# ctu-mrs/space_filling_forest_star

Hardware: AMD Instinct MI355X
Metric: accepted node expansions/sec + collision checks/sec, dense_3D 6-DoF (higher is better)
Workload: dtype f64

## Files before the change

space_filling_forest_star_amd/csrc/forest_dev.cpp:

```cpp
#include <algorithm>
#include <chrono>
#include <cmath>
#include <cstdio>
#include <cstdlib>
#include <cstring>
#include <thread>
#include <vector>

#include "engine.h"
#include "sff_geom.h"

namespace sff {

#define HIPCHK(x) hip_check((x), #x)
using Clock = std::chrono::steady_clock;
static double ms_since(Clock::time_point t0) { return std::chrono::duration<double, std::milli>(Clock::now() - t0).count(); }

static uint64_t next_pow2(uint64_t v) {
  uint64_t p = 1;
  while (p < v) p <<= 1;
  return p;
}

bool Forest::device_eligible() const {
// ... 1573 lines not shown
        if (g[24]) fprintf(stderr, "[sffgpu k_star_tail, sections of a sample's pass (STAR_PASS_TRACE build)] us: first loads %.1f views %.1f evaluate %.1f (of it requests %.1f) "
                           "loops %.1f writes %.1f\n", g[24] / ps / 100.0, g[25] / ps / 100.0, (g[26] + g[27]) / ps / 100.0, g[27] / ps / 100.0, g[28] / ps / 100.0, g[29] / ps / 100.0);
      }
    }
    const double r = (double)std::max<unsigned long long>(1ULL, k.prof[6]);
    if (d.kc_trace.p) {
      const size_t nw = (size_t)cfg.wave / 64 + 2;
      std::vector<unsigned long long> tr(nw * 8);
      HIPCHK(hipMemcpy(tr.data(), d.kc_trace.p, nw * 64, hipMemcpyDeviceToHost));
      unsigned long long t0 = ~0ULL;
      size_t used = 0;
      for (size_t w = 0; w < nw; ++w) if (tr[8 * w]) { t0 = std::min(t0, tr[8 * w]); used = w + 1; }
      static const char* names[8] = {"start", "walk done", "count published", "stamps posted", "lower counts in (ids)", "lower stamps in", "lower owned counts in", "end"};
      for (int k = 0; k < 8 && used; ++k) {
        std::vector<double> v;
        for (size_t w = 0; w < used; ++w) if (tr[8 * w + k]) v.push_back((double)(tr[8 * w + k] - t0) / 100.0);
        if (v.empty()) continue;
        std::vector<double> sv = v;
        std::sort(sv.begin(), sv.end());
        fprintf(stderr, "[sffgpu k_commit trace, %zu workgroups] %-24s us after the first start: min %.1f median %.1f max %.1f | first wg %.1f last wg %.1f\n",
                used, names[k], sv.front(), sv[sv.size() / 2], sv.back(), v.front(), v.back());
      }
    }
    fprintf(stderr, "[sffgpu k_commit us/commit, last workgroup] walks + waits for earlier samples %.1f (%.2f polls, max %llu) "
            "lower workgroups' counts %.1f borders %.1f control block %.1f | dependent/round %.0f\n", k.prof[0] / r / 100.0, k.prof[5] / r,
            (unsigned long long)k.prof[7], k.prof[1] / r / 100.0, k.prof[2] / r / 100.0, k.prof[3] / r / 100.0,
            (double)k.n_unsettled / r);
#ifdef SFFK_CI_TRACE
    {
      std::vector<unsigned long long> tr(4096 * 8);
      sffk::debug_ci_trace(tr.data());
      unsigned long long t0 = ~0ULL, tend = 0;
      for (int w = 0; w < 4096; ++w) if (tr[8 * w]) { t0 = std::min(t0, tr[8 * w]); tend = std::max(tend, tr[8 * w + 7]); }
      struct It { double start, broad, end; int nc, smp, items, wave; double entry, pre; };
      std::vector<It> its;
      int waves = 0, n_pose_items = 0;
      double pose_us = 0, pose_max = 0;
      for (int w = 0; w < 4096; ++w) {
        if (!tr[8 * w]) continue;
        ++waves;
        { const unsigned long long pp = tr[8 * w + 6] >> 8; n_pose_items += (int)(pp & 0xff); pose_us += (double)(pp >> 8) / 100.0; if ((pp & 0xff) && (double)(pp >> 8) / 100.0 > pose_max) pose_max = (double)(pp >> 8) / 100.0; tr[8 * w + 6] &= 0xff; }
        if (!tr[8 * w + 6]) continue;
        its.push_back({(tr[8 * w + 1] - t0) / 100.0, tr[8 * w + 2] >= tr[8 * w + 1] ? (tr[8 * w + 2] - t0) / 100.0 : -1.0, (tr[8 * w + 3] - t0) / 100.0,
                       (int)tr[8 * w + 4], (int)(tr[8 * w + 5] & 0xff), (int)tr[8 * w + 6], w, (tr[8 * w] - t0) / 100.0, ((tr[8 * w + 5] >> 8) - t0) / 100.0});
      }
      std::sort(its.begin(), its.end(), [](const It& a, const It& b) { return a.end > b.end; });
      fprintf(stderr, "[sffgpu k_collide_items trace] %d waves, %zu with items, kernel %.1f us (first start -> last end)\n", waves, its.size(), (tend - t0) / 100.0);
      for (size_t k = 0; k < its.size() && k < 12; ++k)
        fprintf(stderr, "  wave %4d: entry %.1f preamble done %.1f | items %d | first item: start %.1f broad done %.1f end %.1f us | candidates %d masked samples %d\n",
                its[k].wave, its[k].entry, its[k].pre, its[k].items, its[k].start, its[k].broad, its[k].end, its[k].nc, its[k].smp);
      {
        std::vector<double> e, p, st, en;
        for (const It& i : its) { e.push_back(i.entry); p.push_back(i.pre); st.push_back(i.start); en.push_back(i.end); }
        auto q = [](std::vector<double> v, double f) { std::sort(v.begin(), v.end()); return v.empty() ? 0.0 : v[(size_t)(f * (v.size() - 1))]; };
        fprintf(stderr, "  entry min/med/max %.1f %.1f %.1f | preamble done %.1f %.1f %.1f | first item start %.1f %.1f %.1f | end %.1f %.1f %.1f\n",
                q(e, 0), q(e, .5), q(e, 1), q(p, 0), q(p, .5), q(p, 1), q(st, 0), q(st, .5), q(st, 1), q(en, 0), q(en, .5), q(en, 1));
      }
      double sum_b = 0, sum_n = 0; int nb = 0;
      for (const It& i : its) if (i.broad >= 0) { sum_b += i.broad - i.start; sum_n += i.end - i.broad; ++nb; }
      if (nb) fprintf(stderr, "  first items with a broad phase: %d, avg broad %.1f us, avg after-broad %.1f us\n", nb, sum_b / nb, sum_n / nb);
      fprintf(stderr, "  pose items: %d, avg %.1f us, longest per wave %.1f us\n", n_pose_items, n_pose_items ? pose_us / n_pose_items : 0.0, pose_max);
    }
#endif
#ifdef SFFK_DEBUG_COUNTERS
    unsigned long long g[16];
    sffk::debug_counters(g);
    const double items = (double)std::max<unsigned long long>(1ULL, g[1]);
    fprintf(stderr, "[sffgpu exact kernel, per masked chunk] chunks %llu (with work %llu, with candidates %llu) flushes %.2f "
            "candidates %.1f | us: setup %.2f hierarchy %.2f narrow %.2f | per wave total %.1f us over %llu waves\n",
            g[0], g[1], g[2], g[3] / items, g[7] / items, g[4] / items / 100.0, g[5] / items / 100.0, g[6] / items / 100.0,
            (double)g[8] / (double)std::max<unsigned long long>(1ULL, g[9]) / 100.0, g[9]);
    fprintf(stderr, "[sffgpu exact kernel, narrow phase per chunk with candidates] us: staging %.2f culls %.2f exact steps %.2f (the rest: pair formation) | "
            "touching (sample, candidate) pairs %.2f\n", g[10] / 100.0 / (double)std::max<unsigned long long>(1ULL, g[2]),
            g[11] / 100.0 / (double)std::max<unsigned long long>(1ULL, g[2]), g[13] / 100.0 / (double)std::max<unsigned long long>(1ULL, g[2]),
            (double)g[14] / (double)std::max<unsigned long long>(1ULL, g[2]));
    unsigned long long q[16];
    sffk::debug_counters_query(q);
    const double qw = (double)std::max<unsigned long long>(1ULL, q[0]);
    fprintf(stderr, "[sffgpu query kernel, per sampled wave] us: grid scan %.2f classify %.2f cull %.2f (flushes %.2f) | live %.2f "
            "pairs/live %.1f survivors/live %.2f\n", q[1] / qw / 100.0, q[2] / qw / 100.0, q[3] / qw / 100.0, q[4] / qw / 100.0,
            q[7] / qw, (double)q[5] / (double)std::max<unsigned long long>(1ULL, q[7]),
            (double)q[6] / (double)std::max<unsigned long long>(1ULL, q[7]));
    fprintf(stderr, "[sffgpu block query kernel] us per sampled workgroup: samples %.2f | cells+lists %.2f | 2nd list %.2f | exact %.2f | classify %.2f | cull %.2f | flush %.2f\n",
            q[1] / qw / 100.0, q[2] / qw / 100.0, q[3] / qw / 100.0, q[4] / qw / 100.0, q[5] / qw / 100.0, q[6] / qw / 100.0, q[7] / qw / 100.0);
    fprintf(stderr, "[sffgpu block query kernel] shader clock over the sampled workgroups' lifetimes: %.0f MHz (lifetime %.2f us)\n",
            100.0 * (double)q[10] / (double)std::max<unsigned long long>(1ULL, q[11]), q[11] / qw / 100.0);
#endif
  }
}

}
```

space_filling_forest_star_amd/csrc/kernels.hip:

```cpp
#include <hip/hip_runtime.h>
#include <stdint.h>
#include <stdlib.h>
#include <string.h>
#include "kernels.h"
#include <algorithm>
#include "sff_geom.h"
#include "kernels_dev.h"
#include "star_pass_dev.h"
#include "prio_heap_dev.h"

namespace sffk {

using namespace sffg;


__global__ __launch_bounds__(256) void k_sample_steer(SampleLaunch P) {
  const int i = blockIdx.x * blockDim.x + threadIdx.x;
  sample_steer_one(i, P);
}

__device__ __forceinline__ float wrapf(float d) {
  const float PI_F = 3.14159274f;
  if (d < -PI_F) return d + 2.0f * PI_F;
  if (d >= PI_F) return d - 2.0f * PI_F;
// ... 1374 lines not shown
  xform(R, p, rob.center, c);
}

#ifndef SEG_WAVES
#define SEG_WAVES 4
#endif
#ifndef SHARE_WORK
#define SHARE_WORK 192
#endif
#ifndef SHARE_POSE_MIN
#define SHARE_POSE_MIN 8
#endif
#define SHARE_IDLE (1 << 30)
__device__ __forceinline__ int share_block(int nc) { return nc >= 64 ? 4 : (nc >= 24 ? 2 : 1); }
struct ShareSlot {
  unsigned long long sk;
  int nc, done_k, minhit, seg, chunk, kind;
  unsigned long long mask;
  double a[6], b[6], R[9];
};
struct ShareArea {
  ShareSlot slot[SEG_WAVES];
  int done_waves;
};
__device__ __forceinline__ unsigned long long lds_load64(const unsigned long long* p) {
  return __hip_atomic_load(p, __ATOMIC_RELAXED, __HIP_MEMORY_SCOPE_WORKGROUP);
}
__device__ __forceinline__ int lds_load32(const int* p) { return __hip_atomic_load(p, __ATOMIC_RELAXED, __HIP_MEMORY_SCOPE_WORKGROUP); }
__device__ void share_init(ShareArea& sh) {
  if (threadIdx.x < SEG_WAVES) { sh.slot[threadIdx.x].sk = (unsigned long long)SHARE_IDLE; sh.slot[threadIdx.x].nc = 0; }
  if (threadIdx.x == 0) sh.done_waves = 0;
}

__device__ bool pose_block(const EnvView& env, const RobotView& rob, const double* rtri, double* stage, const int32_t* cand,
                           int k0, int kc, const double* p, const double* R, const double* c, double rr, int lane) {
  bool hit = false;
  stage_candidates(env, cand, k0, kc, lane, stage);
  for (int r0 = 0; r0 < rob.n_tri && !hit; r0 += 64) {
    const int r = r0 + lane;
    double Q[9];
    const bool have = r < rob.n_tri;
    if (have)
      for (int v = 0; v < 3; ++v) xform(R, p, rtri + 9 * r + 3 * v, Q + 3 * v);
    bool lane_hit = false;
    for (int k = 0; k < kc; ++k) {
      const double* sb = stage + k * STAGE_TRI;
      if (plane_clear(sb + 6, c, rr)) continue;
      if (have && !lane_hit) {
        if (tri_box_overlap(sb, sb + 3, Q)) lane_hit = sat17(sb + 11, Q);
      }
    }
    hit = __any(lane_hit);
  }
  __builtin_amdgcn_wave_barrier();
  return hit;
}

__device__ bool pose_exact(const EnvView& env, const RobotView& rob, const double* rtri, int32_t* stack, int32_t* cand,
                           double* stage, const double* p, const double* R, const double* c, int lane, ShareArea* share = nullptr) {
  double qlo[3], qhi[3];
  double rr = rob.radius * (1 + 1e-9) + 1e-9 * (fabs(c[0]) + fabs(c[1]) + fabs(c[2]) + 1);
  for (int k = 0; k < 3; ++k) { qlo[k] = c[k] - rr; qhi[k] = c[k] + rr; }

  WaveStack st{stack, 0, stack + STACK_CAP};
  bool overflow;
  int nc = collect_candidates(env, qlo, qhi, lane, st, cand, CAND_CAP, &overflow);
  bool hit = false;
  if (overflow) {
    for (int r0 = 0; r0 < rob.n_tri && !hit; r0 += 64) {
      const int r = r0 + lane;
      double Q[9];
      const bool have = r < rob.n_tri;
      if (have)
        for (int v = 0; v < 3; ++v) xform(R, p, rtri + 9 * r + 3 * v, Q + 3 * v);
      bool lane_hit = false;
      for (int t = 0; t < env.n_tri; ++t) {
        if (have && !lane_hit) {
          const double* b = env.tri_box + 6 * (size_t)t;
          if (tri_box_overlap(b, b + 3, Q)) lane_hit = sat17(env.tri + 9 * (size_t)t, Q);
        }
      }
      hit = __any(lane_hit);
    }
  } else {
    const bool shared = share && nc >= SHARE_POSE_MIN;
    ShareSlot* const hs = shared ? &share->slot[threadIdx.x >> 6] : nullptr;
    unsigned seq = 0;
    if (shared && lane == 0) {
      seq = (unsigned)(hs->sk >> 32) + 1u;
      hs->nc = nc; hs->done_k = 0; hs->minhit = 0x7fffffff; hs->kind = 1;
      for (int k = 0; k < 6; ++k) hs->a[k] = p[k];
      for (int k = 0; k < 3; ++k) hs->b[k] = c[k];
      for (int k = 0; k < 9; ++k) hs->R[k] = R[k];
      __threadfence_block();
      __hip_atomic_store(&hs->sk, (unsigned long long)seq << 32, __ATOMIC_RELAXED, __HIP_MEMORY_SCOPE_WORKGROUP);
    }
    const int blk = shared ? share_block(nc) : STAGE_N;
    for (int knext = 0; !hit; knext += STAGE_N) {
      int k0 = knext;
      if (shared) {
        int seen = 0x7fffffff;
        if (lane == 0) {
          k0 = (int)(unsigned)(atomicAdd(&hs->sk, (unsigned long long)blk) & 0xffffffffULL);
          seen = lds_load32(&hs->minhit);
        }
        k0 = __builtin_amdgcn_readfirstlane(k0);
        seen = __builtin_amdgcn_readfirstlane(seen);
        if (k0 >= nc) break;
        const int kc = nc - k0 < blk ? nc - k0 : blk;
        const bool h = seen == 0 ? true : pose_block(env, rob, rtri, stage, cand, k0, kc, p, R, c, rr, lane);
        if (lane == 0) {
          if (h) atomicMin(&hs->minhit, 0);
          atomicAdd(&hs->done_k, kc);
        }
        continue;
      }
      if (k0 >= nc) break;
      const int kc = nc - k0 < blk ? nc - k0 : blk;
      hit = pose_block(env, rob, rtri, stage, cand, k0, kc, p, R, c, rr, lane);
    }
    if (shared) {
      int out = 0;
      if (lane == 0) {
        while (lds_load32(&hs->done_k) < nc) __builtin_amdgcn_s_sleep(2);
        out = lds_load32(&hs->minhit);
        __hip_atomic_store(&hs->sk, ((unsigned long long)seq << 32) | (unsigned long long)SHARE_IDLE, __ATOMIC_RELAXED, __HIP_MEMORY_SCOPE_WORKGROUP);
      }
      hit = __builtin_amdgcn_readfirstlane(out) == 0;
    }
  }
  return hit;
}

__global__ __launch_bounds__(64 * POSE_WAVES) void k_collide_poses(EnvView env, RobotView rob,
                                                                   const double* __restrict__ pos6, int n,
                                                                   const int32_t* __restrict__ live_flags,
                                                                   uint8_t* __restrict__ hit_out, int explicit_rt) {
  extern __shared__ double lds_d[];
  double* rtri = lds_d;
  const int wave = threadIdx.x >> 6, lane = threadIdx.x & 63;
  double* stage = rtri + (size_t)rob.n_tri * 9 + (size_t)wave * STAGE_DOUBLES;
  int32_t* ibase = reinterpret_cast<int32_t*>(rtri + (size_t)rob.n_tri * 9 + (size_t)POSE_WAVES * STAGE_DOUBLES);
  int32_t* stack = ibase + wave * (STACK_CAP + TG_HASH);
  int32_t* cand = ibase + POSE_WAVES * (STACK_CAP + TG_HASH) + wave * CAND_CAP;
  const int pose = blockIdx.x * POSE_WAVES + wave;
  bool need = false;
  double p[6], R[9], c[3] = {0, 0, 0};
  if (pose < n) {
    const bool run = !live_flags || (live_flags[pose] & 3) == 1;
    if (run && env.n_tri != 0) {
      if (explicit_rt) {
        const double* rt = pos6 + 12 * (size_t)pose;
        for (int k = 0; k < 9; ++k) R[k] = rt[k];
        for (int k = 0; k < 3; ++k) { p[k] = rt[9 + k]; p[3 + k] = 0; }
        need = !surely_clear(env, p);
        if (need) xform(R, p, rob.center, c);
      } else {
        for (int k = 0; k < 6; ++k) p[k] = pos6[6 * (size_t)pose + k];
        need = !surely_clear(env, p);
        if (need) pose_frame(rob, pos6, pose, p, R, c);
      }
    }
    if (!need && lane == 0) hit_out[pose] = 0;
  }
  if (!__syncthreads_or(need ? 1 : 0)) return;
  for (int i = threadIdx.x; i < rob.n_tri * 9; i += blockDim.x) rtri[i] = rob.tri[i];
  __syncthreads();
  if (!need) return;
  const bool hit = pose_exact(env, rob, rtri, stack, cand, stage, p, R, c, lane);
  if (lane == 0) hit_out[pose] = hit ? 1 : 0;
}

__device__ __forceinline__ void fill_robot_boxes(const double* rtri, double* rbox, int n_tri, int tid, int nthreads) {
  for (int r = tid; r < n_tri; r += nthreads)
    for (int ax = 0; ax < 3; ++ax) {
      rbox[6 * r + ax] = min3(rtri[9 * r + ax], rtri[9 * r + 3 + ax], rtri[9 * r + 6 + ax]);
      rbox[6 * r + 3 + ax] = max3(rtri[9 * r + ax], rtri[9 * r + 3 + ax], rtri[9 * r + 6 + ax]);
    }
}

#define QUEUE_CAP 128

struct SegLane {
  double a[3], dir[3], parts;
  int s0;
  int idx;
  bool need;
  double P[3], C[3], rr;
};
__device__ int narrow_block(const EnvView& env, const RobotView& rob, const double* rtri, const double* rbox, int32_t* queue,
                            double* stage, const int32_t* cand, int k0, int kc, const SegLane& L, int minhit, int lane DBG_ARG) {
  const double* a = L.a; const double* dir = L.dir;
  const double parts = L.parts;
  const int s0 = L.s0;
  const int idx = L.idx;
  const bool need = L.need;
  const double* P = L.P; const double* C = L.C;
  const double rr = L.rr;
  int qn = 0;
  auto flush = [&](int count) {
    DBG_ADD(3, 1);
    [[maybe_unused]] const unsigned long long tf_ = DBG_T();
    int v = 0x7fffffff;
    if (lane < count) {
      const int e = queue[lane];
      const int sl = e & 63, r = (e >> 6) & 1023, k = e >> 16;
      const int sidx = s0 + sl;
      if (sidx < minhit) {
        double S[3], Q[9];
        edge_sample_pos(a, dir, parts, sidx, S);
        for (int vv = 0; vv < 3; ++vv)
          for (int ax = 0; ax < 3; ++ax) Q[3 * vv + ax] = rtri[9 * r + 3 * vv + ax] + S[ax];
        if (sat17(stage + k * STAGE_TRI + 11, Q)) v = sidx;
      }
// ... 73 lines not shown
  while (true) {
    bool worked = false;
    for (int w2 = 0; w2 < SEG_WAVES; ++w2) {
      if (w2 == wave) continue;
      ShareSlot& hs = sh.slot[w2];
      int k0 = SHARE_IDLE, nc = 0, blk = 1;
      if (lane == 0) {
        const unsigned long long cur = lds_load64(&hs.sk);
        const int nc0 = lds_load32(&hs.nc);
        if ((int)(unsigned)(cur & 0xffffffffULL) < nc0) {
          blk = share_block(nc0);
          k0 = (int)(unsigned)(atomicAdd(&hs.sk, (unsigned long long)blk) & 0xffffffffULL);
          __threadfence_block();
          nc = lds_load32(&hs.nc);
        }
      }
      __threadfence_block();
      k0 = __builtin_amdgcn_readfirstlane(k0);
      nc = __builtin_amdgcn_readfirstlane(nc);
      blk = __builtin_amdgcn_readfirstlane(blk);
      if (k0 >= nc) continue;
      worked = true;
      const int kc = nc - k0 < blk ? nc - k0 : blk;
      int mh = 0;
      if (lane == 0) mh = lds_load32(&hs.minhit);
      mh = __builtin_amdgcn_readfirstlane(mh);
      if (hs.kind == 1) {
        if (mh != 0) {
          double pp[6], RR[9], cc[3];
          for (int k = 0; k < 6; ++k) pp[k] = hs.a[k];
          for (int k = 0; k < 3; ++k) cc[k] = hs.b[k];
          for (int k = 0; k < 9; ++k) RR[k] = hs.R[k];
          const double rr = rob.radius * (1 + 1e-9) + 1e-9 * (fabs(cc[0]) + fabs(cc[1]) + fabs(cc[2]) + 1);
          if (pose_block(env, rob, rtri, stage, cand_base + w2 * CAND_CAP, k0, kc, pp, RR, cc, rr, lane)) mh = 0;
        }
      } else {
        double a[6], b[6];
        for (int k = 0; k < 6; ++k) { a[k] = hs.a[k]; b[k] = hs.b[k]; }
        const unsigned long long mask = hs.mask;
        const int chunk = hs.chunk;
        SegLane L;
        L.parts = edge_parts(a, b);
        L.s0 = 1 + 64 * chunk;
        for (int k = 0; k < 3; ++k) { L.a[k] = a[k]; L.dir[k] = b[k] - a[k]; L.P[k] = 0.0; }
        L.idx = L.s0 + lane;
        L.need = ((mask >> lane) & 1ULL) != 0;
        if (L.idx <= edge_samples(L.parts)) edge_sample_pos(L.a, L.dir, L.parts, L.idx, L.P);
        for (int k = 0; k < 3; ++k) L.C[k] = L.P[k] + rob.center[k];
        L.rr = rob.radius * (1 + 1e-9) + 1e-9 * (fabs(L.C[0]) + fabs(L.C[1]) + fabs(L.C[2]) + 1);
        mh = narrow_block(env, rob, rtri, rbox, queue, stage, cand_base + w2 * CAND_CAP, k0, kc, L, mh, lane DBG_PASS);
      }
      __builtin_amdgcn_wave_barrier();
      if (lane == 0) {
        if (mh != 0x7fffffff) atomicMin(&hs.minhit, mh);
        __threadfence_block();
        atomicAdd(&hs.done_k, kc);
      }
    }
    if (!worked) {
      int dw = 0;
      if (lane == 0) dw = lds_load32(&sh.done_waves);
      if (__builtin_amdgcn_readfirstlane(dw) >= SEG_WAVES) break;
      __builtin_amdgcn_s_sleep(20);
    }
  }
}

// ... 275 lines not shown
  DBG_DECL
  [[maybe_unused]] const unsigned long long tk_ = DBG_T();
  const int W = gridDim.x * SEG_WAVES;
  const int w0 = blockIdx.x + gridDim.x * wave;
  __shared__ int pool_n, pool_next;
  __shared__ int pool_e[64 * SEG_WAVES];
  __shared__ unsigned long long pool_m[64 * SEG_WAVES];
  auto pool_put = [&](bool s, int e, unsigned long long m) {
    const unsigned long long bal = __ballot(s);
    int off = 0;
    if (lane == 0 && bal) off = atomicAdd(&pool_n, __popcll(bal));
    off = __shfl(off, 0);
    if (s) {
      const int at = off + __popcll(bal & ((1ULL << lane) - 1ULL));
      pool_e[at] = e;
      pool_m[at] = m;
    }
  };
  auto pool_take = [&]() -> int {
    int i = 0;
    if (lane == 0) i = atomicAdd(&pool_next, 1);
    return __shfl(i, 0);
  };
  for (int base = 0; base < n_pose; base += 64 * W) {
    if (threadIdx.x == 0) { pool_n = 0; pool_next = 0; }
    __syncthreads();
    const int mine = base + w0 + W * lane;
    pool_put(mine < n_pose && pose_hit[mine] == 2, mine, 0ULL);
    __syncthreads();
    for (int i = pool_take(); i < pool_n; i = pool_take()) {
      const int pose = pool_e[i];
      double p[6], R[9], c[3];
      pose_frame(rob, pos6, pose, p, R, c);
      const bool hit = pose_exact(env, rob, rtri, stack, cand, stage, p, R, c, lane);
      if (lane == 0) pose_hit[pose] = hit ? 1 : 0;
    }
    __syncthreads();
  }
  if (!ctrl[3]) {
    const int M = ctrl[2];
    for (int base = 0; base < M; base += 64 * W) {
      if (threadIdx.x == 0) { pool_n = 0; pool_next = 0; }
      __syncthreads();
      const int mine = base + w0 + W * lane;
      const unsigned long long m = mine < M ? masks[(size_t)base + (size_t)w0 * 64 + lane] : 0ULL;
      pool_put(m != 0ULL, mine, m);
      __syncthreads();
      for (int i = pool_take(); i < pool_n; i = pool_take()) {
        const int e = pool_e[i];
        const unsigned long long nm = pool_m[i];
        const int slot = list[e].slot, chunk = list[e].chunk;
        if (chunk > 0 && first_hit[slot] <= 64 * chunk) continue;
        double a[6], b[6];
        for (int k = 0; k < 6; ++k) { a[k] = a6[6 * (size_t)slot + k]; b[k] = b6[6 * (size_t)slot + k]; }
        segment_chunk(env, rob, rtri, rbox, stack, cand, queue, stage, a, b, slot, chunk, true, nm, first_hit, overflow_flag, lane DBG_PASS);
      }
      __syncthreads();
    }
    DBG_ADD(8, DBG_T() - tk_);
    DBG_ADD(9, 1);
    DBG_FLUSH();
    return;
  }
  while (true) {
    int first = 0;
    if (lane == 0) first = atomicAdd(ctrl + 1, 64);
    first = __shfl(first, 0);
// ... 1190 lines not shown
    unsigned long long mask = 0ULL;
    if (!ran_over) {
      size_t at;
      if (e < MH) {
        const int sl = __popcll(__ballot(sub_incl <= e));
        at = (size_t)sl * sub_cap + (e - (__shfl(sub_incl, sl) - __shfl(sub_n, sl)));
      } else {
        const int e2 = e - MH;
        const int sl = __popcll(__ballot(sub_incl_l <= e2));
        at = (size_t)sl * sub_cap + sub_half + (e2 - (__shfl(sub_incl_l, sl) - __shfl(sub_nl, sl)));
      }
      const SurvivorItem it = list[at];
      slot = it.slot; c_lo = it.chunk; c_hi = it.chunk + 1; mask = it.mask;
    } else if (e < n_pose) {
      if ((live_flags[e] & 3) != 1) continue;
      slot = -1 - e; c_lo = c_hi = 0;
    } else {
      slot = e - n_pose;
      if (D.on) {
        const int si = slot / stride;
        if ((live_flags[si] & 3) != 1 || slot - si * stride > D.rec_nnb[si]) continue;
      }
      const int ns = seg_ns[slot];
      if (ns <= 0) continue;
      c_lo = 0; c_hi = (ns + 63) >> 6;
    }
    if (slot < 0) {
      const int pose = -1 - slot;
      double p[6], R[9], c[3];
#ifdef SFFK_CI_TRACE
      const unsigned long long ci_p0 = wall_clock64();
#endif
      pose_frame(rob, pos6, pose, p, R, c);
      const bool hit = pose_exact(env, rob, rtri, stack, cand, stage, p, R, c, lane, (SHARE && !ran_over) ? &s_share : nullptr);
      if (lane == 0) pose_hit[pose] = hit ? 1 : 0;
#ifdef SFFK_CI_TRACE
      ci_first[3] += ((wall_clock64() - ci_p0) << 8) | 1ULL;
#endif
      continue;
    }
    double a[6], b[6];
    if (D.on && ran_over) {
      const int si = slot / stride, t = slot - si * stride;
      const double* pe = D.center ? D.center + 6 * (size_t)si : D.pos + 6 * (size_t)D.parent[si];
      const double* pq = pos6 + 6 * (size_t)si;
      if (t == 0) { for (int k = 0; k < 6; ++k) { a[k] = pe[k]; b[k] = pq[k]; } }
      else {
        const int id = D.rec_nb[(size_t)si * D.nbcap + t - 1];
        const bool same = (D.rec_meta[(size_t)si * D.nbcap + t - 1] & 1) != 0;
        const double* pn = D.pos + 6 * (size_t)id;
        if (same) { for (int k = 0; k < 6; ++k) { a[k] = pn[k]; b[k] = pq[k]; } }
        else if (id == D.goal_id) { for (int k = 0; k < 6; ++k) { a[k] = pq[k]; b[k] = pn[k]; } }
        else { for (int k = 0; k < 6; ++k) { a[k] = pe[k]; b[k] = pn[k]; } }
      }
    } else {
      for (int k = 0; k < 6; ++k) { a[k] = a6[6 * (size_t)slot + k]; b[k] = b6[6 * (size_t)slot + k]; }
    }
    for (int chunk = c_lo; chunk < c_hi; ++chunk) {
      if (chunk > 0 && first_hit[slot] <= 64 * chunk) break;
#ifdef SFFK_CI_TRACE
      const unsigned long long ci_a = wall_clock64();
#endif
      segment_chunk(env, rob, rtri, rbox, stack, cand, queue, stage, a, b, slot, chunk, !ran_over, mask, first_hit, overflow_flag, lane DBG_PASS,
                            (SHARE && !ran_over) ? &s_share : nullptr);
#ifdef SFFK_CI_TRACE
      if (ci_items == 0) { ci_first[0] = ci_a; ci_first[1] = wall_clock64(); ci_first[2] = (unsigned long long)__popcll(mask); }
      ++ci_items;
// ... 423 lines not shown
        }
      }
      uint32_t word[4];
#pragma unroll
      for (int u = 0; u < 4; ++u) word[u] = wp[u] ? *wp[u] : 0u;
      unsigned long long m0, m1, m2, m3;
      {
        unsigned long long mm[4];
#pragma unroll
        for (int u = 0; u < 4; ++u) {
          if (wp[u] && ((word[u] >> sh[u]) & 1u)) need[u] = false;
          mm[u] = __ballot(need[u]);
        }
        m0 = mm[0]; m1 = mm[1]; m2 = mm[2]; m3 = mm[3];
      }
      for (int u = 0; u < 4 && fh == 0x7fffffff; ++u) {
        const unsigned long long mask = u == 0 ? m0 : (u == 1 ? m1 : (u == 2 ? m2 : m3));
        if (mask == 0ULL) continue;
        segment_chunk(env, rob, rtri, rbox, stack, cand, queue, stage, a, b, 0, c0 + u, true, mask, fh_lds, ovf_lds, lane DBG_PASS);
        __builtin_amdgcn_wave_barrier();
        fh = *fh_lds;
        if (*ovf_lds) {
          __builtin_amdgcn_wave_barrier();
          if (lane == 0) { *fh_lds = 0x7fffffff; *ovf_lds = 0; }
          __builtin_amdgcn_wave_barrier();
          fh = 0x7fffffff;
          const double dir[3] = {b[0] - a[0], b[1] - a[1], b[2] - a[2]};
          const int last = 64 * (c0 + u) + 64 < ns ? 64 * (c0 + u) + 64 : ns;
          for (int idx = 1 + 64 * (c0 + u); idx <= last && fh == 0x7fffffff; ++idx) {
            double P[6] = {0, 0, 0, 0, 0, 0}, Rm[9] = {1, 0, 0, 0, 1, 0, 0, 0, 1}, c3[3];
            edge_sample_pos(a, dir, parts, idx, P);
            if (surely_clear_edge(env, P)) continue;
            xform(Rm, P, rob.center, c3);
            if (pose_exact(env, rob, rtri, stack, cand, stage, P, Rm, c3, lane)) fh = idx;
          }
        }
      }
    }
  }
  calls += fh == 0x7fffffff ? (unsigned long long)ns : (unsigned long long)fh;
  return fh == 0x7fffffff;
}

__device__ __attribute__((noinline)) void sq_knn(const GridView& g, const double* qp, int tree, int k, int tcnt, double cell_edge, double slack, int lane,
                       TopK& t, int& have, int max_id = 0x7fffffff, const int32_t* give_up = nullptr, uint32_t step = 0,
                       unsigned long long* dbg = nullptr, const int32_t* lds_cancel = nullptr, int job = 0) {
  t.d = 1.0e300; t.id = 0x7fffffff;
  have = 0;
  unsigned long long d_sh = 0, d_ob = 0, d_cg = 0, d_in = 0;
  if (k <= 0) return;
  const int k_store = k < tcnt ? k : tcnt;
  auto offer = [&](bool valid, const GridItem* src) {
    bool cand = false;
    double d = 1.0e300;
    int id = 0x7fffffff;
    if (valid) {
      const unsigned long long* q8 = reinterpret_cast<const unsigned long long*>(src);
      unsigned long long pw[6];
      for (int q = 0; q < 6; ++q) pw[q] = sq_u64(q8 + q);
      const unsigned long long it = sq_u64(q8 + 6);
      id = (int)(unsigned)(it & 0xffffffffULL);
      if ((int)(unsigned)(it >> 32) == tree && id < max_id) {
        double p6[6];
        for (int q = 0; q < 6; ++q) p6[q] = __longlong_as_double((long long)pw[q]);
        d = dist6(p6, qp);
        cand = true;
      }
// ... 933 lines not shown
      {
        uint32_t v = 0;
        for (int k = 0; k < 6; ++k) { v = lane == 2 * k ? sp_lo(qp[k]) : v; v = lane == 2 * k + 1 ? sp_hi(qp[k]) : v; }
        v = lane == 12 ? (uint32_t)mine : v;
        v = lane == 13 ? sp_lo(best) : v; v = lane == 14 ? sp_hi(best) : v;
        v = lane == 15 ? (ok ? 1u : 0u) : v;
        if (lane < 16) wt_u64(my_rec + SFFK_SPEC_EARLY + lane, sp_gran(step, v));
      }
      bool flt = false, reject = true;
      int kstar = 0;
      if (OPT) kstar = __popcll(__ballot(lane > 0 && lane <= SFFK_STAR_KMAX + 1 && A.ktab[lane] <= snn));
      if (ok) {
        if (lane == 0) {
          for (int k = 0; k < 6; ++k) j_qp[k] = qp[k];
          j_pdist = pdist;
          lds_st(&j_mine, mine); lds_st(&j_k, kstar); lds_st(&j_nn0, nns); lds_st(&j_snn, snn); lds_st(&j_step, (int)step);
        }
        ++myseq;
        __builtin_amdgcn_fence(__ATOMIC_RELEASE, "workgroup");
        if (lane == 0) lds_st(&j_seq, myseq);
      }
      auto helper_wait = [&](const int32_t* word, int want) {
        while (lds_ld(word) < want) __builtin_amdgcn_s_sleep(1);
        __builtin_amdgcn_fence(__ATOMIC_ACQUIRE, "workgroup");
      };
      if (ok) {
        cc_l += 1; ex_pose += 1;
        bool hit = false;
        if (A.env.n_tri != 0 && !surely_clear(A.env, qp)) {
          double Rm[9], c3[3];
          if (qp[3] == 0 && qp[4] == 0 && qp[5] == 0) { Rm[0] = Rm[4] = Rm[8] = 1; Rm[1] = Rm[2] = Rm[3] = Rm[5] = Rm[6] = Rm[7] = 0; }
          else rotation(qp, Rm);
          xform(Rm, qp, A.rob.center, c3);
          hit = pose_exact(A.env, A.rob, rtri, stack, cand, stage, qp, Rm, c3, lane);
        }
        beat(2);
        if (!hit) {
          pf_l += 1; ex_seg += 1;
          const bool free0 = (sq_edge_clear_fast(A.env, cpos, qp, lane, cc_l, ex_smp) || sq_path_free(A.env, A.rob, rtri, stack, cand, queue, stage, cpos, qp, &s_fh, &s_ovf, lane, cc_l, ex_smp, flt));
          reject = !free0;
          beat(3);
          if (!reject && stale()) aborted = true;
          int n_hit = 0;
          if (!flt && !reject && !aborted) {
            nq_l += R;
            const double r = pdist > A.dist_tree ? pdist : A.dist_tree;
            helper_wait(&j_done, myseq);
            n_hit = lds_ld(&j_nhit);
            for (int p = 0; p < n_pend; ++p) {
              double pp[6];
              for (int k = 0; k < 6; ++k) pp[k] = p_pos[6 * p + k];
              const double d = dist6(pp, qp);
              if (d < r) {
                if (lane == 0 && n_hit < 64) {
                  h_id[n_hit] = nns + p; h_tree[n_hit] = p_tree[p]; h_d[n_hit] = d;
                  for (int k = 0; k < 6; ++k) h_pos[6 * n_hit + k] = pp[k];
                }
                ++n_hit;
              }
            }
            for (int p = 0; p < na && !aborted; ++p) {
              const unsigned long long* ep = S.rec + ((size_t)set * S.n_slots + pslot[p]) * SFFK_SPEC_REC + SFFK_SPEC_EARLY;
              SP_WAVE_SYNC();
              for (int spin = 0;; ++spin) {
                const unsigned long long g2 = sq_u64(ep + (lane & 15));
                if (__all((uint32_t)(g2 >> 32) == step)) { s_row[lane] = (uint32_t)g2; break; }
                if ((spin & 15) == 15 && stale()) { aborted = true; break; }
// ... 653 lines not shown
```

space_filling_forest_star_amd/csrc/rrt_seq_batch.inc:

```

__device__ __attribute__((noinline)) void rrt_knn_sweep(const NodeStoreMut& st, int n, const double* qp, int tree, int k, int lane, TopK& t,
                                                        int& have) {
  t.d = 1.0e300; t.id = 0x7fffffff;
  have = 0;
  if (k <= 0) return;
  for (int base = 0; base < n; base += 256) {
    int tr[4];
#pragma unroll
    for (int u = 0; u < 4; ++u) {
      const int j = base + 64 * u + lane;
      tr[u] = j < n ? sq_i32(st.tree + j) : -1;
    }
    unsigned long long pw[4][6];
#pragma unroll
    for (int u = 0; u < 4; ++u) {
      const int j = base + 64 * u + lane;
      if (tr[u] == tree) {
        const unsigned long long* q8 = reinterpret_cast<const unsigned long long*>(st.pos + 6 * (size_t)j);
        for (int q = 0; q < 6; ++q) pw[u][q] = sq_u64(q8 + q);
      }
    }
#pragma unroll
    for (int u = 0; u < 4; ++u) {
      if (base + 64 * u >= n) continue;
// ... 75 lines not shown
      rnd[0] = x; rnd[1] = y; rnd[2] = 0; rnd[3] = rnd[4] = rnd[5] = 0;
      if (A.dim == 6) {
        rnd[2] = uniform_real(A.ring[cursor & A.ring_mask], A.limits[4], A.limits[5]);
        rnd[3] = uniform_real(A.ring[(cursor + 1) & A.ring_mask], -SFFG_PI, SFFG_PI);
        double phi = sffp::pacos(sample_acos_arg(A.ring[(cursor + 2) & A.ring_mask])) + SFFG_PI_2;
        if (uniform_real(A.ring[(cursor + 3) & A.ring_mask], 0.0, 1.0) < 0.5) { if (phi < 0) phi += SFFG_PI; else phi -= SFFG_PI; }
        rnd[4] = phi;
        rnd[5] = uniform_real(A.ring[(cursor + 4) & A.ring_mask], -SFFG_PI, SFFG_PI);
        cursor += 5;
      }
    }
    nq += 1;
    TopK nt{1.0e300, 0x7fffffff};
    int n_near = 0;
    knn(rnd, mine, merged() ? 2 : 1, nt, n_near);
    if (n_near < 1) { hand_over(SFFK_RRT_WHY_CAPACITY); break; }
    if constexpr (!LAZY) {
      if (n_near >= 2 && __shfl(nt.d, 0) == __shfl(nt.d, 1)) { hand_over(SFFK_RRT_WHY_TIE); break; }
    }
    int nearest = __shfl(nt.id, 0);
    double cpos[6], qp[6];
    for (int k = 0; k < 6; ++k) cpos[k] = sq_f64(A.st.pos + 6 * (size_t)nearest + k);
    steer(cpos, rnd, A.sampling_dist, qp);
    bool nan = false;
    for (int k = 0; k < 6; ++k) nan = nan || !(qp[k] == qp[k]);
    if (nan) { hand_over(SFFK_RRT_WHY_DEGENERATE); break; }
    cc += 1;
    bool hit = false;
    if (A.env.n_tri != 0 && !surely_clear(A.env, qp)) {
      double Rm[9], c3[3];
      if (qp[3] == 0 && qp[4] == 0 && qp[5] == 0) { Rm[0] = Rm[4] = Rm[8] = 1; Rm[1] = Rm[2] = Rm[3] = Rm[5] = Rm[6] = Rm[7] = 0; }
      else rotation(qp, Rm);
      xform(Rm, qp, A.rob.center, c3);
      hit = pose_exact(A.env, A.rob, rtri, stack, cand, stage, qp, Rm, c3, lane);
    }
    if (hit) continue;
    bool flt = false;
    pf += 1;
    if (!(sq_edge_clear_fast(A.env, cpos, qp, lane, cc, ex_smp) || sq_path_free(A.env, A.rob, rtri, stack, cand, queue, stage, cpos, qp, &s_fh, &s_ovf, lane, cc, ex_smp, flt))) continue;
    if constexpr (!LAZY) if (n_live > 1) {
      nq += (unsigned long long)(n_live - 1);
      const double r = A.dist_tree;
      const double ri = (r + A.sweep_abs_eps) * (1.0 + 1e-5);
      const float rf = sqrtf((float)(ri * ri) * 1.000001f) * 1.000001f;
      const float qx = (float)qp[0], qy = (float)qp[1], qz = (float)qp[2];
      const int lx = grid_coord(qx - rf, g.ox, g.inv_cell, g.nx), hx = grid_coord(qx + rf, g.ox, g.inv_cell, g.nx);
      const int ly = grid_coord(qy - rf, g.oy, g.inv_cell, g.ny), hy = grid_coord(qy + rf, g.oy, g.inv_cell, g.ny);
      const int lz = grid_coord(qz - rf, g.oz, g.inv_cell, g.nz), hz = grid_coord(qz + rf, g.oz, g.inv_cell, g.nz);
      const int wx = hx - lx + 1, wy = hy - ly + 1, wz = hz - lz + 1;
      const int total = wx * wy * wz;
      double bd = 1.0e300;
      int bid = 0x7fffffff;
      bool btie = false;
      auto take = [&](bool valid, const GridItem* src) {
        bool h = false;
        double d = 0;
        int id = 0, tr = 0;
        if (valid) {
          const unsigned long long* q8 = reinterpret_cast<const unsigned long long*>(src);
          double p6[6];
          for (int k = 0; k < 6; ++k) p6[k] = __longlong_as_double((long long)sq_u64(q8 + k));
          const unsigned long long w = sq_u64(q8 + 6);
          id = (int)(unsigned)(w & 0xffffffffULL); tr = (int)(unsigned)(w >> 32);
          d = dist6(p6, qp);
          h = tr != mine && d < r;
        }
        unsigned long long hm = __ballot(h);
// ... 163 lines not shown
```

space_filling_forest_star_amd/csrc/seq_waves_body.inc:

```
  extern __shared__ double lds_d[];
  __shared__ int32_t s_fh, s_ovf;
  __shared__ int32_t h_id[64], h_tree[64];
  __shared__ double h_d[64], h_pos[64 * 6];
  const DevForestView& f = A.f;
  DevCtrl* c = f.ctrl;
  const int lane = threadIdx.x;
  if (c->halt || c->in_wave) return;
  __shared__ int32_t p_size[PRIO ? SFFK_PRIO_MAX_HEAPS : 1];
  __shared__ int32_t p_tne[PRIO ? 64 : 1];
  double* rtri = lds_d;
  double* stage = rtri + (size_t)A.rob.n_tri * 9;
  int32_t* ibase = reinterpret_cast<int32_t*>(stage + STAGE_DOUBLES);
  int32_t* stack = ibase;
  int32_t* cand = ibase + (STACK_CAP + TG_HASH);
  int32_t* queue = cand + CAND_CAP;
  for (int i = lane; i < A.rob.n_tri * 9; i += 64) rtri[i] = A.rob.tri[i];
  __builtin_amdgcn_wave_barrier();
  fill_robot_boxes(rtri, reinterpret_cast<double*>(queue + QUEUE_CAP), A.rob.n_tri, lane, 64);
  __builtin_amdgcn_wave_barrier();
  int n_nodes = c->n_nodes, iter = c->iter, fn = c->frontier_n, cn = c->closed_n, nb = c->n_borders;
  int solved = c->solved, empty_frontier = c->empty_frontier, terminated = c->terminated;
  const int front_sel = c->front_sel;
  unsigned long long cursor = c->cursor, cc = c->collide_calls, pf = c->path_free_calls, nq = c->nn_queries;
  unsigned long long ex_pose = c->poses_executed, ex_seg = c->segments_executed, ex_smp = c->samples_executed;
// ... 99 lines not shown
      pre_at = cursor + (unsigned long long)WP;
      for (int k = 0; k < 6; ++k) pre_w[k] = k < WP ? f.ring[(pre_at + k) & f.ring_mask] : 0ULL;
      SampleTrig ht{};
      if (A.trig) {
        const double* t0 = A.trig + 3 * (size_t)(cursor & f.ring_mask);
        ht.c_phi = t0[0]; ht.s_phi = t0[1];
        if (WP == 6) {
          const double* t1 = A.trig + 3 * (size_t)((cursor + 1) & f.ring_mask);
          const double* t3 = A.trig + 3 * (size_t)((cursor + 3) & f.ring_mask);
          ht.c_theta = t1[0]; ht.s_theta = t1[1]; ht.acos_u = t3[2];
        }
      }
      cursor += (unsigned long long)WP;
      ++iter;
      ++rounds; rnodes += (unsigned long long)(n_nodes + 1); ++rqueries;
      double qp[6];
      if (!A.trig) {
        const double ang = sample_angle(lane == 1 ? w[1] : w[0]);
        const double sv = sffp::psin(ang), cv = sffp::pcos(ang);
        ht.s_phi = __shfl(sv, 0); ht.c_phi = __shfl(cv, 0);
        ht.s_theta = __shfl(sv, 1); ht.c_theta = __shfl(cv, 1);
        ht.acos_u = WP == 6 ? sffp::pacos(sample_acos_arg(w[3])) : 0.0;
      }
      const bool ok = sample_point_with(w, cpos, A.sampling_dist, A.dim, A.limits, qp, ht);
      lap(1);
      if (!ok) continue;
      cc += 1; ex_pose += 1;
      bool hit = false;
      if (A.env.n_tri != 0 && !surely_clear(A.env, qp)) {
        double Rm[9], c3[3];
        if (qp[3] == 0 && qp[4] == 0 && qp[5] == 0) { Rm[0] = Rm[4] = Rm[8] = 1; Rm[1] = Rm[2] = Rm[3] = Rm[5] = Rm[6] = Rm[7] = 0; }
        else rotation(qp, Rm);
        xform(Rm, qp, A.rob.center, c3);
        hit = pose_exact(A.env, A.rob, rtri, stack, cand, stage, qp, Rm, c3, lane);
      }
      lap(2);
      if (hit) continue;
      pf += 1; ex_seg += 1;
      const bool free0 = (sq_edge_clear_fast(A.env, cpos, qp, lane, cc, ex_smp) || sq_path_free(A.env, A.rob, rtri, stack, cand, queue, stage, cpos, qp, &s_fh, &s_ovf, lane, cc, ex_smp, flt));
      bool reject = !free0;
      lap(3);
      const double pdist = dist6(cpos, qp);
      int n_hit = 0;
      [[maybe_unused]] bool solving = false;
      [[maybe_unused]] double gpos[6] = {0, 0, 0, 0, 0, 0};
      if (!flt && !reject) {
        nq += (unsigned long long)R;
        const double r = pdist > A.dist_tree ? pdist : A.dist_tree;
        const double ri = (r + A.sweep_abs_eps) * (1.0 + 1e-5);
        const float rf = sqrtf((float)(ri * ri) * 1.000001f) * 1.000001f;
        const GridView& g = A.g;
        const float qx = (float)qp[0], qy = (float)qp[1], qz = (float)qp[2];
        const int lx = grid_coord(qx - rf, g.ox, g.inv_cell, g.nx), hx = grid_coord(qx + rf, g.ox, g.inv_cell, g.nx);
        const int ly = grid_coord(qy - rf, g.oy, g.inv_cell, g.ny), hy = grid_coord(qy + rf, g.oy, g.inv_cell, g.ny);
        const int lz = grid_coord(qz - rf, g.oz, g.inv_cell, g.nz), hz = grid_coord(qz + rf, g.oz, g.inv_cell, g.nz);
        const int wx = hx - lx + 1, wy = hy - ly + 1, wz = hz - lz + 1;
        const int total = wx * wy * wz;
        auto take = [&](bool valid, const GridItem* src) {
          bool h = false;
          double d = 0, p6[6];
          int id = 0, tr = 0;
          if (valid) {
            const unsigned long long* q8 = reinterpret_cast<const unsigned long long*>(src);
            for (int k = 0; k < 6; ++k) p6[k] = __longlong_as_double((long long)sq_u64(q8 + k));
            const unsigned long long it = sq_u64(q8 + 6);
            id = (int)(unsigned)(it & 0xffffffffULL); tr = (int)(unsigned)(it >> 32);
            d = dist6(p6, qp);
// ... 342 lines not shown
```

Baseline: 11.35 million.

## Compact pose-block robot/candidate pairs into a wave queue before exact SAT tests

The pose collision block previously had each lane loop over all staged candidates for its own robot triangle, running the exact SAT test divergently. It now computes each robot triangle's AABB, ballots the (candidate, triangle) pairs that pass the box test, compacts them into a per-wave LDS queue, and flushes 64 pairs at a time so all lanes run the SAT test together. This is meant to cut lane divergence in the narrow phase, at the cost of extra ballots, LDS queue traffic and recomputing the triangle transform at flush time. It also threads a queue pointer through every pose_exact caller, allocates a queue region in the pose kernel's LDS layout, and adds tail-wave trace output to the debug path.

```diff
diff --git a/profiles/compare_dumps.py b/profiles/compare_dumps.py
--- /dev/null
+++ b/profiles/compare_dumps.py
@@ -0,0 +1,11 @@
+import os
+import sys
+
+import numpy as np
+
+a, b = sys.argv[1:3]
+names = sorted(os.listdir(a))
+assert names == sorted(os.listdir(b)) and names, (names, sorted(os.listdir(b)))
+for n in names:
+    assert np.array_equal(np.load(os.path.join(a, n)), np.load(os.path.join(b, n))), n
+print("dump-outputs: %d files equal" % len(names))
diff --git a/space_filling_forest_star_amd/csrc/forest_dev.cpp b/space_filling_forest_star_amd/csrc/forest_dev.cpp
--- a/space_filling_forest_star_amd/csrc/forest_dev.cpp
+++ b/space_filling_forest_star_amd/csrc/forest_dev.cpp
@@ -1629,17 +1629,20 @@
       sffk::debug_ci_trace(tr.data());
       unsigned long long t0 = ~0ULL, tend = 0;
       for (int w = 0; w < 4096; ++w) if (tr[8 * w]) { t0 = std::min(t0, tr[8 * w]); tend = std::max(tend, tr[8 * w + 7]); }
-      struct It { double start, broad, end; int nc, smp, items, wave; double entry, pre; };
-      std::vector<It> its;
+      struct It { double start, broad, end; int nc, smp, items, wave; double entry, pre; int poses; double pose_us, last; };
+      std::vector<It> its, tails;
       int waves = 0, n_pose_items = 0;
       double pose_us = 0, pose_max = 0;
       for (int w = 0; w < 4096; ++w) {
         if (!tr[8 * w]) continue;
         ++waves;
-        { const unsigned long long pp = tr[8 * w + 6] >> 8; n_pose_items += (int)(pp & 0xff); pose_us += (double)(pp >> 8) / 100.0; if ((pp & 0xff) && (double)(pp >> 8) / 100.0 > pose_max) pose_max = (double)(pp >> 8) / 100.0; tr[8 * w + 6] &= 0xff; }
-        if (!tr[8 * w + 6]) continue;
+        const unsigned long long pp = tr[8 * w + 6] >> 8;
+        { n_pose_items += (int)(pp & 0xff); pose_us += (double)(pp >> 8) / 100.0; if ((pp & 0xff) && (double)(pp >> 8) / 100.0 > pose_max) pose_max = (double)(pp >> 8) / 100.0; tr[8 * w + 6] &= 0xff; }
+        if (!tr[8 * w + 6]) { if (pp & 0xff) tails.push_back({0, -1.0, 0, 0, 0, 0, w, (tr[8 * w] - t0) / 100.0, 0, (int)(pp & 0xff), (double)(pp >> 8) / 100.0, (tr[8 * w + 7] - t0) / 100.0}); continue; }
         its.push_back({(tr[8 * w + 1] - t0) / 100.0, tr[8 * w + 2] >= tr[8 * w + 1] ? (tr[8 * w + 2] - t0) / 100.0 : -1.0, (tr[8 * w + 3] - t0) / 100.0,
-                       (int)tr[8 * w + 4], (int)(tr[8 * w + 5] & 0xff), (int)tr[8 * w + 6], w, (tr[8 * w] - t0) / 100.0, ((tr[8 * w + 5] >> 8) - t0) / 100.0});
+                       (int)tr[8 * w + 4], (int)(tr[8 * w + 5] & 0xff), (int)tr[8 * w + 6], w, (tr[8 * w] - t0) / 100.0, ((tr[8 * w + 5] >> 8) - t0) / 100.0,
+                       (int)(pp & 0xff), (double)(pp >> 8) / 100.0, (tr[8 * w + 7] - t0) / 100.0});
+        tails.push_back(its.back());
       }
       std::sort(its.begin(), its.end(), [](const It& a, const It& b) { return a.end > b.end; });
       fprintf(stderr, "[sffgpu k_collide_items trace] %d waves, %zu with items, kernel %.1f us (first start -> last end)\n", waves, its.size(), (tend - t0) / 100.0);
@@ -1657,6 +1660,17 @@
       for (const It& i : its) if (i.broad >= 0) { sum_b += i.broad - i.start; sum_n += i.end - i.broad; ++nb; }
       if (nb) fprintf(stderr, "  first items with a broad phase: %d, avg broad %.1f us, avg after-broad %.1f us\n", nb, sum_b / nb, sum_n / nb);
       fprintf(stderr, "  pose items: %d, avg %.1f us, longest per wave %.1f us\n", n_pose_items, n_pose_items ? pose_us / n_pose_items : 0.0, pose_max);
+      std::sort(tails.begin(), tails.end(), [](const It& a, const It& b) { return a.last > b.last; });
+      int with_pose = 0;
+      double tail_pose = 0;
+      for (size_t k = 0; k < tails.size() && k < 32; ++k) {
+        with_pose += tails[k].poses > 0;
+        tail_pose += tails[k].pose_us;
+        fprintf(stderr, "  tail %2zu: wave %4d left at %.1f us | chunks %d | pose items %d, %.1f us\n", k, tails[k].wave, tails[k].last, tails[k].items,
+                tails[k].poses, tails[k].pose_us);
+      }
+      fprintf(stderr, "  last 32 wavefronts: %d with a pose item, %.1f us of pose items on average among those\n", with_pose,
+              with_pose ? tail_pose / with_pose : 0.0);
     }
 #endif
 #ifdef SFFK_DEBUG_COUNTERS
diff --git a/space_filling_forest_star_amd/csrc/kernels.hip b/space_filling_forest_star_amd/csrc/kernels.hip
--- a/space_filling_forest_star_amd/csrc/kernels.hip
+++ b/space_filling_forest_star_amd/csrc/kernels.hip
@@ -1430,32 +1430,65 @@
   if (threadIdx.x == 0) sh.done_waves = 0;
 }
 
-__device__ bool pose_block(const EnvView& env, const RobotView& rob, const double* rtri, double* stage, const int32_t* cand,
-                           int k0, int kc, const double* p, const double* R, const double* c, double rr, int lane) {
+#define QUEUE_CAP 128
+static_assert(STAGE_N <= 64, "a pose pair's queue entry keeps the stage index in six bits");
+
+__device__ bool pose_block(const EnvView& env, const RobotView& rob, const double* rtri, double* stage, int32_t* queue,
+                           const int32_t* cand, int k0, int kc, const double* p, const double* R, const double* c, double rr,
+                           int lane) {
   bool hit = false;
+  int qn = 0;
+  auto flush = [&](int count) {
+    bool h = false;
+    if (lane < count) {
+      const int e = queue[lane];
+      const int k = e & 63, r = e >> 6;
+      double Q[9];
+      for (int v = 0; v < 3; ++v) xform(R, p, rtri + 9 * r + 3 * v, Q + 3 * v);
+      h = sat17(stage + k * STAGE_TRI + 11, Q);
+    }
+    hit = __any(h);
+    int keep = 0;
+    if (lane + count < qn) keep = queue[lane + count];
+    if (lane + count < qn) queue[lane] = keep;
+    qn -= count;
+  };
   stage_candidates(env, cand, k0, kc, lane, stage);
   for (int r0 = 0; r0 < rob.n_tri && !hit; r0 += 64) {
     const int r = r0 + lane;
-    double Q[9];
     const bool have = r < rob.n_tri;
-    if (have)
+    double qmin[3] = {0, 0, 0}, qmax[3] = {0, 0, 0};
+    if (have) {
+      double Q[9];
       for (int v = 0; v < 3; ++v) xform(R, p, rtri + 9 * r + 3 * v, Q + 3 * v);
-    bool lane_hit = false;
-    for (int k = 0; k < kc; ++k) {
+      for (int ax = 0; ax < 3; ++ax) {
+        qmin[ax] = min3(Q[ax], Q[3 + ax], Q[6 + ax]);
+        qmax[ax] = max3(Q[ax], Q[3 + ax], Q[6 + ax]);
+      }
+    }
+    for (int k = 0; k < kc && !hit; ++k) {
       const double* sb = stage + k * STAGE_TRI;
-      if (plane_clear(sb + 6, c, rr)) continue;
-      if (have && !lane_hit) {
-        if (tri_box_overlap(sb, sb + 3, Q)) lane_hit = sat17(sb + 11, Q);
-      }
-    }
-    hit = __any(lane_hit);
+      if (!plane_clear(sb + 6, c, rr)) {
+        bool ok = have;
+        for (int ax = 0; ax < 3; ++ax)
+          if (sb[ax] > qmax[ax] || qmin[ax] > sb[3 + ax]) ok = false;
+        const unsigned long long mm = __ballot(ok);
+        if (mm) {
+          const int before = __popcll(mm & ((1ULL << lane) - 1ULL));
+          if (ok) queue[qn + before] = k | (r << 6);
+          qn += __popcll(mm);
+        }
+      }
+      const bool last = k + 1 == kc && r0 + 64 >= rob.n_tri;
+      while (!hit && (qn >= 64 || (last && qn > 0))) flush(qn < 64 ? qn : 64);
+    }
   }
   __builtin_amdgcn_wave_barrier();
   return hit;
 }
 
 __device__ bool pose_exact(const EnvView& env, const RobotView& rob, const double* rtri, int32_t* stack, int32_t* cand,
-                           double* stage, const double* p, const double* R, const double* c, int lane, ShareArea* share = nullptr) {
+                           int32_t* queue, double* stage, const double* p, const double* R, const double* c, int lane, ShareArea* share = nullptr) {
   double qlo[3], qhi[3];
   double rr = rob.radius * (1 + 1e-9) + 1e-9 * (fabs(c[0]) + fabs(c[1]) + fabs(c[2]) + 1);
   for (int k = 0; k < 3; ++k) { qlo[k] = c[k] - rr; qhi[k] = c[k] + rr; }
@@ -1506,7 +1539,7 @@
         seen = __builtin_amdgcn_readfirstlane(seen);
         if (k0 >= nc) break;
         const int kc = nc - k0 < blk ? nc - k0 : blk;
-        const bool h = seen == 0 ? true : pose_block(env, rob, rtri, stage, cand, k0, kc, p, R, c, rr, lane);
+        const bool h = seen == 0 ? true : pose_block(env, rob, rtri, stage, queue, cand, k0, kc, p, R, c, rr, lane);
         if (lane == 0) {
           if (h) atomicMin(&hs->minhit, 0);
           atomicAdd(&hs->done_k, kc);
@@ -1515,7 +1548,7 @@
       }
       if (k0 >= nc) break;
       const int kc = nc - k0 < blk ? nc - k0 : blk;
-      hit = pose_block(env, rob, rtri, stage, cand, k0, kc, p, R, c, rr, lane);
+      hit = pose_block(env, rob, rtri, stage, queue, cand, k0, kc, p, R, c, rr, lane);
     }
     if (shared) {
       int out = 0;
@@ -1541,6 +1574,7 @@
   int32_t* ibase = reinterpret_cast<int32_t*>(rtri + (size_t)rob.n_tri * 9 + (size_t)POSE_WAVES * STAGE_DOUBLES);
   int32_t* stack = ibase + wave * (STACK_CAP + TG_HASH);
   int32_t* cand = ibase + POSE_WAVES * (STACK_CAP + TG_HASH) + wave * CAND_CAP;
+  int32_t* queue = ibase + POSE_WAVES * (STACK_CAP + TG_HASH + CAND_CAP) + wave * QUEUE_CAP;
   const int pose = blockIdx.x * POSE_WAVES + wave;
   bool need = false;
   double p[6], R[9], c[3] = {0, 0, 0};
@@ -1565,7 +1599,7 @@
   for (int i = threadIdx.x; i < rob.n_tri * 9; i += blockDim.x) rtri[i] = rob.tri[i];
   __syncthreads();
   if (!need) return;
-  const bool hit = pose_exact(env, rob, rtri, stack, cand, stage, p, R, c, lane);
+  const bool hit = pose_exact(env, rob, rtri, stack, cand, queue, stage, p, R, c, lane);
   if (lane == 0) hit_out[pose] = hit ? 1 : 0;
 }
 
@@ -1576,8 +1610,6 @@
       rbox[6 * r + 3 + ax] = max3(rtri[9 * r + ax], rtri[9 * r + 3 + ax], rtri[9 * r + 6 + ax]);
     }
 }
-
-#define QUEUE_CAP 128
 
 struct SegLane {
   double a[3], dir[3], parts;
@@ -1717,7 +1749,7 @@
           for (int k = 0; k < 3; ++k) cc[k] = hs.b[k];
           for (int k = 0; k < 9; ++k) RR[k] = hs.R[k];
           const double rr = rob.radius * (1 + 1e-9) + 1e-9 * (fabs(cc[0]) + fabs(cc[1]) + fabs(cc[2]) + 1);
-          if (pose_block(env, rob, rtri, stage, cand_base + w2 * CAND_CAP, k0, kc, pp, RR, cc, rr, lane)) mh = 0;
+          if (pose_block(env, rob, rtri, stage, queue, cand_base + w2 * CAND_CAP, k0, kc, pp, RR, cc, rr, lane)) mh = 0;
         }
       } else {
         double a[6], b[6];
@@ -2059,7 +2091,7 @@
       const int pose = pool_e[i];
       double p[6], R[9], c[3];
       pose_frame(rob, pos6, pose, p, R, c);
-      const bool hit = pose_exact(env, rob, rtri, stack, cand, stage, p, R, c, lane);
+      const bool hit = pose_exact(env, rob, rtri, stack, cand, queue, stage, p, R, c, lane);
       if (lane == 0) pose_hit[pose] = hit ? 1 : 0;
     }
     __syncthreads();
@@ -3316,7 +3348,7 @@
       const unsigned long long ci_p0 = wall_clock64();
 #endif
       pose_frame(rob, pos6, pose, p, R, c);
-      const bool hit = pose_exact(env, rob, rtri, stack, cand, stage, p, R, c, lane, (SHARE && !ran_over) ? &s_share : nullptr);
+      const bool hit = pose_exact(env, rob, rtri, stack, cand, queue, stage, p, R, c, lane, (SHARE && !ran_over) ? &s_share : nullptr);
       if (lane == 0) pose_hit[pose] = hit ? 1 : 0;
 #ifdef SFFK_CI_TRACE
       ci_first[3] += ((wall_clock64() - ci_p0) << 8) | 1ULL;
@@ -3806,7 +3838,7 @@
             edge_sample_pos(a, dir, parts, idx, P);
             if (surely_clear_edge(env, P)) continue;
             xform(Rm, P, rob.center, c3);
-            if (pose_exact(env, rob, rtri, stack, cand, stage, P, Rm, c3, lane)) fh = idx;
+            if (pose_exact(env, rob, rtri, stack, cand, queue, stage, P, Rm, c3, lane)) fh = idx;
           }
         }
       }
@@ -4806,7 +4838,7 @@
           if (qp[3] == 0 && qp[4] == 0 && qp[5] == 0) { Rm[0] = Rm[4] = Rm[8] = 1; Rm[1] = Rm[2] = Rm[3] = Rm[5] = Rm[6] = Rm[7] = 0; }
           else rotation(qp, Rm);
           xform(Rm, qp, A.rob.center, c3);
-          hit = pose_exact(A.env, A.rob, rtri, stack, cand, stage, qp, Rm, c3, lane);
+          hit = pose_exact(A.env, A.rob, rtri, stack, cand, queue, stage, qp, Rm, c3, lane);
         }
         beat(2);
         if (!hit) {
diff --git a/space_filling_forest_star_amd/csrc/rrt_seq_batch.inc b/space_filling_forest_star_amd/csrc/rrt_seq_batch.inc
--- a/space_filling_forest_star_amd/csrc/rrt_seq_batch.inc
+++ b/space_filling_forest_star_amd/csrc/rrt_seq_batch.inc
@@ -131,7 +131,7 @@
       if (qp[3] == 0 && qp[4] == 0 && qp[5] == 0) { Rm[0] = Rm[4] = Rm[8] = 1; Rm[1] = Rm[2] = Rm[3] = Rm[5] = Rm[6] = Rm[7] = 0; }
       else rotation(qp, Rm);
       xform(Rm, qp, A.rob.center, c3);
-      hit = pose_exact(A.env, A.rob, rtri, stack, cand, stage, qp, Rm, c3, lane);
+      hit = pose_exact(A.env, A.rob, rtri, stack, cand, queue, stage, qp, Rm, c3, lane);
     }
     if (hit) continue;
     bool flt = false;
diff --git a/space_filling_forest_star_amd/csrc/seq_waves_body.inc b/space_filling_forest_star_amd/csrc/seq_waves_body.inc
--- a/space_filling_forest_star_amd/csrc/seq_waves_body.inc
+++ b/space_filling_forest_star_amd/csrc/seq_waves_body.inc
@@ -155,7 +155,7 @@
         if (qp[3] == 0 && qp[4] == 0 && qp[5] == 0) { Rm[0] = Rm[4] = Rm[8] = 1; Rm[1] = Rm[2] = Rm[3] = Rm[5] = Rm[6] = Rm[7] = 0; }
         else rotation(qp, Rm);
         xform(Rm, qp, A.rob.center, c3);
-        hit = pose_exact(A.env, A.rob, rtri, stack, cand, stage, qp, Rm, c3, lane);
+        hit = pose_exact(A.env, A.rob, rtri, stack, cand, queue, stage, qp, Rm, c3, lane);
       }
       lap(2);
       if (hit) continue;
```

Result: no change. 11.26 million (-0.8%).
